# kvas7andy/unreal

Hardware: AMD Instinct MI355X
Metric: env-steps/sec (whole node), UNREAL maze 84x84 (higher is better)
Workload: dtype f32 (fp16x2-split MFMA operands, fp32 accumulate)

## Files before the change

unreal_amd/csrc/gemm_split.hip:

```cpp
#include "common.h"

namespace {

constexpr int BK = 32;
constexpr int NPL = 2;
typedef _Float16 f16x8 __attribute__((ext_vector_type(8)));
typedef _Float16 f16x2 __attribute__((ext_vector_type(2)));
constexpr int ROW_B = 80;
constexpr int FLAG_RELU = 1, FLAG_ACCUM = 2, FLAG_ATOMIC = 4, FLAG_RELU_MASK = 8, FLAG_RELU_BITS = 16;

typedef float f32x2 __attribute__((ext_vector_type(2)));
typedef unsigned int u32x2 __attribute__((ext_vector_type(2)));
typedef unsigned int u32x4 __attribute__((ext_vector_type(4)));

__device__ __forceinline__ int row_deal(int j) { return (j & ~7) | ((j & 1) << 2) | ((j >> 1) & 3); }

struct SplitArgs {
  int M, N, K;
  const float* A; int lda;
  const unsigned short* W; int ldw; long plane;
  float* C; int ldc;
  const float* bias;
  const float* mask; int ldm;
  int flags;
  int vecA;
  int nbx, nby;
  int splitk, ktiles_per_split;
  long slab_stride;
  const float* c_prev; float* c_out; float* h_out; int ld_h;
  const float* A2; int lda2, K1, K1pad;
  const float* dh_above; float* dc_io; const float* gates_act; const float* c_new; float* dpre;
  const float* a_absmax; float a_floor; const float* w_absmax; float* c_absmax0; float* c_absmax1;
};

template <int ROWS, bool VEC>
__device__ __forceinline__ f32x4 a_piece_load(const float* __restrict__ P, int ld, int rows_total, int K, int r0, int k0, int p,
                                              int tid) {
  const int id = tid + 256 * p;
  const int r = min(r0 + row_deal(id / (BK / 4)), rows_total - 1);
  const int k = k0 + (id % (BK / 4)) * 4;
  const float* row = P + (size_t)r * ld;
  if (VEC) return *reinterpret_cast<const f32x4*>(row + min(k, ld - 4));
  f32x4 v;
#pragma unroll
  for (int e = 0; e < 4; ++e) v[e] = row[min(k + e, K - 1)];
  return v;
}

__device__ __forceinline__ void split4_terms(float x0, float x1, float x2, float x3, u32x2 (&pl)[NPL]) {
  const f16x2 h01 = __builtin_convertvector((f32x2){x0, x1}, f16x2), h23 = __builtin_convertvector((f32x2){x2, x3}, f16x2);
  const f32x2 r01 = (f32x2){x0, x1} - __builtin_convertvector(h01, f32x2), r23 = (f32x2){x2, x3} - __builtin_convertvector(h23, f32x2);
  const f16x2 l01 = __builtin_convertvector(r01, f16x2), l23 = __builtin_convertvector(r23, f16x2);
  pl[0] = (u32x2){__builtin_bit_cast(unsigned int, h01), __builtin_bit_cast(unsigned int, h23)};
  pl[1] = (u32x2){__builtin_bit_cast(unsigned int, l01), __builtin_bit_cast(unsigned int, l23)};
}

template <int ROWS>
__device__ __forceinline__ void a_piece_store(unsigned char* S, f32x4 v, int klim, int p, int tid, float scale) {
  const int id = tid + 256 * p;
  const int r = row_deal(id / (BK / 4)), k = (id % (BK / 4)) * 4;
#pragma unroll
  for (int e = 0; e < 4; ++e) v[e] = k + e < klim ? v[e] * scale : 0.f;
  u32x2 pl[NPL];
  split4_terms(v[0], v[1], v[2], v[3], pl);
#pragma unroll
  for (int t = 0; t < NPL; ++t)
    *reinterpret_cast<u32x2*>(S + (t * ROWS + r) * ROW_B + k * 2) = pl[t];
}

template <int ROWS>
__device__ __forceinline__ u32x4 w_piece_load(const unsigned short* __restrict__ W, int ldw, long plane, int rows_total,
                                              int r0, int k0, int p, int tid) {
  const int id = tid + 256 * p;
  const int t = id / (ROWS * 4), r = row_deal((id / 4) % ROWS), c = id % 4;
  const int row = min(r0 + r, rows_total - 1);
  return *reinterpret_cast<const u32x4*>(W + t * plane + (size_t)row * ldw + k0 + c * 8);
}

template <int ROWS>
__device__ __forceinline__ void w_piece_store(unsigned char* S, u32x4 v, int p, int tid) {
  const int id = tid + 256 * p;
  const int t = id / (ROWS * 4), r = row_deal((id / 4) % ROWS), c = id % 4;
  *reinterpret_cast<u32x4*>(S + (t * ROWS + r) * ROW_B + c * 16) = v;
}

template <int BM, int BN, bool SWZ = false>
__device__ __forceinline__ void read_frags(const unsigned char* As, const unsigned char* Bs, int wm, int wn, int li, int kh,
                                           int ks, f16x8 (&af)[BM / 64][NPL], f16x8 (&bf)[BN / 64][NPL]) {
  const int c = 2 * ks + kh;
#pragma unroll
  for (int i = 0; i < BM / 64; ++i)
#pragma unroll
    for (int t = 0; t < NPL; ++t) {
      const int r = wm * (BM / 2) + i * 32 + li;
      af[i][t] = *reinterpret_cast<const f16x8*>(As + (t * BM + r) * ROW_B + (SWZ ? (c ^ ((r >> 4) & 3)) : c) * 16);
    }
#pragma unroll
  for (int j = 0; j < BN / 64; ++j)
#pragma unroll
    for (int t = 0; t < NPL; ++t) {
      const int r = wn * (BN / 2) + j * 32 + li;
      bf[j][t] = *reinterpret_cast<const f16x8*>(Bs + (t * BN + r) * ROW_B + (SWZ ? (c ^ ((r >> 4) & 3)) : c) * 16);
    }
}

template <int TM, int TN>
__device__ __forceinline__ void mma_frags(const f16x8 (&af)[TM][NPL], const f16x8 (&bf)[TN][NPL], f32x16 (&acc)[TM][TN]) {
#pragma unroll
  for (int i = 0; i < TM; ++i)
#pragma unroll
    for (int j = 0; j < TN; ++j) {
      f32x16 c = acc[i][j];
      c = __builtin_amdgcn_mfma_f32_32x32x16_f16(af[i][1], bf[j][0], c, 0, 0, 0);
      c = __builtin_amdgcn_mfma_f32_32x32x16_f16(af[i][0], bf[j][1], c, 0, 0, 0);
      c = __builtin_amdgcn_mfma_f32_32x32x16_f16(af[i][0], bf[j][0], c, 0, 0, 0);
      acc[i][j] = c;
    }
}

template <bool DUAL>
struct ASrc { const float* P; int ld, K, k0; };

template <bool DUAL>
__device__ __forceinline__ ASrc<DUAL> a_src(const SplitArgs& p, int kg) {
  ASrc<DUAL> s;
  if (DUAL) {
    const bool second = kg >= p.K1pad;
    s.P = second ? p.A2 : p.A; s.ld = second ? p.lda2 : p.lda;
    s.K = second ? p.K - p.K1pad : p.K1; s.k0 = second ? kg - p.K1pad : kg;
  } else {
    s.P = p.A; s.ld = p.lda; s.K = p.K; s.k0 = kg;
  }
  return s;
}

template <int BM, int BN, bool VEC, int EPI = 0, int KW = 1, bool DUAL = false>
__global__ __launch_bounds__(256 * KW, KW == 1 ? ((BM == 128 && EPI == 0) ? 3 : 2) : 1) void gemm_split_nt_kernel(SplitArgs p) {
  constexpr bool DEEP = BM == 64;
  constexpr int TM = BM / 64, TN = BN / 64;
  constexpr int PA = BM * BK / 1024, PW = NPL * BN / 64;
  constexpr int A_BYTES = NPL * BM * ROW_B, B_BYTES = NPL * BN * ROW_B;
  const float SA = pow2_scale(fmaxf(p.a_absmax ? *p.a_absmax : 0.f, p.a_floor));
  const float INV_A = pow2_inv(SA);
  const float INV_W = pow2_inv(pow2_scale(*p.w_absmax));
  constexpr bool HALF = BM == 128 && EPI == 0 && KW == 1;
  constexpr int C_BYTES = (HALF ? BM / 2 : BM) * (BN + 4) * 4;
  constexpr int OP_BYTES = A_BYTES + B_BYTES;
  constexpr int RED_BYTES = 64;
  constexpr int SMEM = OP_BYTES > (C_BYTES + RED_BYTES) ? OP_BYTES : (C_BYTES + RED_BYTES);
  static_assert(4 * KW * 4 <= RED_BYTES, "one float per wave");
  __shared__ __attribute__((aligned(16))) unsigned char smem_all[KW * SMEM];
  const int tid = KW == 1 ? (int)threadIdx.x : (int)(threadIdx.x & 255);
  const int grp = KW == 1 ? 0 : (int)(threadIdx.x >> 8);
  unsigned char* smem = smem_all + grp * SMEM;
  unsigned char* As = smem;
  unsigned char* Bs = smem + A_BYTES;

  const int L = blockIdx.x, xcd = L & 7, s = L >> 3;
  const int slab = s % p.splitk, s2 = s / p.splitk;
  const int bx = s2 % p.nbx, by = (s2 / p.nbx) * 8 + xcd;
  if (by >= p.nby) return;
  const int m0 = by * BM, n0 = bx * BN;
  if (EPI == 0) p.C += (size_t)slab * p.slab_stride;
  const int kt_base = slab * p.ktiles_per_split;
  const int nkt = min((p.K + BK - 1) / BK - kt_base, p.ktiles_per_split);
  if (nkt <= 0) return;
  const int lane = tid & 63, wave = tid >> 6;
  const int wm = wave >> 1, wn = wave & 1;
  const int li = lane & 31, kh = lane >> 5;

  f32x16 acc[TM][TN];
#pragma unroll
  for (int i = 0; i < TM; ++i)
#pragma unroll
    for (int j = 0; j < TN; ++j)
#pragma unroll
      for (int r = 0; r < 16; ++r) acc[i][j][r] = 0.f;

  f32x4 ra[2][PA];
  u32x4 rw[PW];
  const int shift = (int)((unsigned)by * 7u % (unsigned)nkt);
#define KT_AT(i) (kt_base + (((i) + shift) >= nkt ? (i) + shift - nkt : (i) + shift))
#define KG_AT(i) (KT_AT(min((i) * KW + grp, nkt - 1)) * BK)
#define KLIM(i, src) ((KW == 1 || (i) * KW + grp < nkt) ? (src).K - (src).k0 : 0)
#define A_LOAD(src, q) a_piece_load<BM, VEC>((src).P, (src).ld, p.M, (src).K, m0, (src).k0, q, tid)
  const int nit = (nkt + KW - 1) / KW;
  {
    const int k0 = KG_AT(0);
    const ASrc<DUAL> s0 = a_src<DUAL>(p, k0);
#pragma unroll
    for (int q = 0; q < PA; ++q) ra[0][q] = A_LOAD(s0, q);
#pragma unroll
    for (int q = 0; q < PW; ++q) rw[q] = w_piece_load<BN>(p.W, p.ldw, p.plane, p.N, n0, k0, q, tid);
#pragma unroll
    for (int q = 0; q < PA; ++q) a_piece_store<BM>(As, ra[0][q], KLIM(0, s0), q, tid, SA);
#pragma unroll
    for (int q = 0; q < PW; ++q) w_piece_store<BN>(Bs, rw[q], q, tid);
    const int k1 = KG_AT(1), k2 = KG_AT(2);
    const ASrc<DUAL> s1 = a_src<DUAL>(p, k1), s2_ = a_src<DUAL>(p, k2);
#pragma unroll
    for (int q = 0; q < PA; ++q) ra[0][q] = A_LOAD(s1, q);
    if (DEEP) {
#pragma unroll
      for (int q = 0; q < PA; ++q) ra[1][q] = A_LOAD(s2_, q);
    }
#pragma unroll
    for (int q = 0; q < PW; ++q) rw[q] = w_piece_load<BN>(p.W, p.ldw, p.plane, p.N, n0, k1, q, tid);
  }
  __syncthreads();

#define SPLIT_NT_TILE(S, IT)                                                                                        \
  {                                                                                                                 \
    f16x8 af[TM][NPL], bf[TN][NPL];                                                                                 \
    read_frags<BM, BN>(As, Bs, wm, wn, li, kh, 0, af, bf);                                                          \
    mma_frags<TM, TN>(af, bf, acc);                                                                                 \
    read_frags<BM, BN>(As, Bs, wm, wn, li, kh, 1, af, bf);          \
    __syncthreads();                                                               \
    const int kcur = KG_AT((IT) + 1), kw = KG_AT((IT) + 2), ka = KG_AT((IT) + (DEEP ? 3 : 2));                      \
    const ASrc<DUAL> scur = a_src<DUAL>(p, kcur), snext = a_src<DUAL>(p, ka);                                       \
    const int klim = KLIM((IT) + 1, scur);                                                                          \
    _Pragma("unroll") for (int q = 0; q < PA; ++q) {                                                                \
      a_piece_store<BM>(As, ra[S][q], klim, q, tid, SA);                                                            \
      ra[S][q] = A_LOAD(snext, q);                                                                                  \
    }                                                                                                               \
    _Pragma("unroll") for (int q = 0; q < PW; ++q) {                                                                \
      w_piece_store<BN>(Bs, rw[q], q, tid);                                                                         \
      rw[q] = w_piece_load<BN>(p.W, p.ldw, p.plane, p.N, n0, kw, q, tid);                                           \
    }                                                                                                               \
    mma_frags<TM, TN>(af, bf, acc);                                                                                 \
    __syncthreads();                                                                    \
  }
  if (DEEP) {
    for (int it = 0; it < nit; it += 2) {
      SPLIT_NT_TILE(0, it)
      if (it + 1 < nit) SPLIT_NT_TILE(1, it + 1)
    }
  } else {
    for (int it = 0; it < nit; ++it) SPLIT_NT_TILE(0, it)
  }
#undef SPLIT_NT_TILE
#undef A_LOAD
#undef KLIM
#undef KG_AT
#undef KT_AT

  if (EPI == 0 && (p.flags & FLAG_ATOMIC)) {
#pragma unroll
    for (int i = 0; i < TM; ++i)
#pragma unroll
      for (int j = 0; j < TN; ++j) {
        const int col = n0 + wn * (BN / 2) + j * 32 + li;
        if (col >= p.N) continue;
        const float bv = (p.bias && slab == 0 && grp == 0) ? p.bias[col] : 0.f;
#pragma unroll
        for (int r = 0; r < 16; ++r) {
          const int row = m0 + wm * (BM / 2) + i * 32 + (r & 3) + 8 * (r >> 2) + 4 * kh;
          const float v = (acc[i][j][r] * INV_A) * INV_W;
          if (row < p.M) atomicAdd(p.C + (size_t)row * p.ldc + col, v + bv);
        }
      }
    return;
  }
  constexpr int CLD = BN + 4;
  float* Cs = reinterpret_cast<float*>(smem);
  if (HALF) {
    const uint16_t* mbits = reinterpret_cast<const uint16_t*>(p.mask);
    const bool vecC = ((p.ldc & 3) == 0) && ((((uintptr_t)p.C) & 15) == 0) &&
                      (!p.bias || ((((uintptr_t)p.bias) & 15) == 0)) &&
                      (!(p.flags & FLAG_RELU_MASK) || (((p.ldm & 3) == 0) && ((((uintptr_t)p.mask) & 15) == 0)));
    constexpr int CV = BN / 4;
    float omax = 0.f;
#pragma unroll 1
    for (int half = 0; half < 2; ++half) {
      if (half) __syncthreads();
      if (wm == half) {
#pragma unroll
        for (int i = 0; i < TM; ++i)
#pragma unroll
          for (int j = 0; j < TN; ++j)
#pragma unroll
            for (int r = 0; r < 16; ++r)
              Cs[(i * 32 + (r & 3) + 8 * (r >> 2) + 4 * kh) * CLD + wn * (BN / 2) + j * 32 + li] =
                  (acc[i][j][r] * INV_A) * INV_W;
      }
      __syncthreads();
      for (int id = threadIdx.x; id < (BM / 2) * CV; id += 256) {
        const int r = id / CV, c4 = (id % CV) * 4;
        const int row = m0 + half * (BM / 2) + r, col = n0 + c4;
        if (row >= p.M || col >= p.N) continue;
        f32x4 v = *reinterpret_cast<const f32x4*>(Cs + r * CLD + c4);
        float* cp = p.C + (size_t)row * p.ldc + col;
        if (vecC && col + 3 < p.N) {
          if (p.bias) { const f32x4 b4 = *reinterpret_cast<const f32x4*>(p.bias + col); v += b4; }
          if (p.flags & FLAG_ACCUM) v += *reinterpret_cast<const f32x4*>(cp);
          if (p.flags & FLAG_RELU) {
#pragma unroll
            for (int e = 0; e < 4; ++e) v[e] = fmaxf(v[e], 0.f);
          }
          if (p.flags & FLAG_RELU_MASK) {
            const f32x4 m4 = *reinterpret_cast<const f32x4*>(p.mask + (size_t)row * p.ldm + col);
#pragma unroll
            for (int e = 0; e < 4; ++e) v[e] = m4[e] > 0.f ? v[e] : 0.f;
          }
          if (p.flags & FLAG_RELU_BITS) {
            const unsigned w = mbits[(size_t)row * p.ldm + (col >> 4)] >> (col & 15);
#pragma unroll
            for (int e = 0; e < 4; ++e) v[e] = ((w >> e) & 1u) ? v[e] : 0.f;
          }
          *reinterpret_cast<f32x4*>(cp) = v;
          omax = fmaxf(fmaxf(omax, fmaxf(fabsf(v[0]), fabsf(v[1]))), fmaxf(fabsf(v[2]), fabsf(v[3])));
        } else {
#pragma unroll
          for (int e = 0; e < 4; ++e) {
            if (col + e >= p.N) break;
            float x = v[e] + (p.bias ? p.bias[col + e] : 0.f);
            if (p.flags & FLAG_ACCUM) x += cp[e];
            if (p.flags & FLAG_RELU) x = fmaxf(x, 0.f);
            if (p.flags & FLAG_RELU_MASK) x = (p.mask[(size_t)row * p.ldm + col + e] > 0.f) ? x : 0.f;
            if (p.flags & FLAG_RELU_BITS) x = ((mbits[(size_t)row * p.ldm + ((col + e) >> 4)] >> ((col + e) & 15)) & 1u) ? x : 0.f;
            cp[e] = x;
            omax = fmaxf(omax, fabsf(x));
          }
        }
      }
    }
    if (p.c_absmax0) {
      __syncthreads();
      float* wmx0 = reinterpret_cast<float*>(smem_all);
      omax = wave_max(omax);
      if ((threadIdx.x & 63) == 0) wmx0[threadIdx.x >> 6] = omax;
      __syncthreads();
      if (threadIdx.x < 64) absmax_commit(p.c_absmax0, fmaxf(fmaxf(wmx0[0], wmx0[1]), fmaxf(wmx0[2], wmx0[3])));
    }
    return;
  }
#pragma unroll
  for (int i = 0; i < TM; ++i)
#pragma unroll
    for (int j = 0; j < TN; ++j)
#pragma unroll
      for (int r = 0; r < 16; ++r)
        Cs[(wm * (BM / 2) + i * 32 + (r & 3) + 8 * (r >> 2) + 4 * kh) * CLD + wn * (BN / 2) + j * 32 + li] =
            (acc[i][j][r] * INV_A) * INV_W;
  __syncthreads();
  const float* C0 = reinterpret_cast<const float*>(smem_all);
  constexpr int GSTRIDE = SMEM / 4;
  if (EPI == 1) {
    const int u0 = bx * (BN / 4);
    const bool add_pre = (p.flags & FLAG_ACCUM) != 0;
    constexpr int ITEMS = BM * (BN / 4) / (256 * KW);
    float cprev[ITEMS], pre4[ITEMS][4];
#pragma unroll
    for (int e = 0; e < ITEMS; ++e) {
      const int id = threadIdx.x + e * 256 * KW;
      const int row = min(m0 + id / (BN / 4), p.M - 1), u = u0 + id % (BN / 4);
      cprev[e] = p.c_prev[(size_t)row * 256 + u];
#pragma unroll
      for (int g4 = 0; g4 < 4; ++g4) pre4[e][g4] = add_pre ? p.C[(size_t)row * p.ldc + g4 * 256 + u] : 0.f;
    }
    static_assert((256 * KW) % (BN / 4) == 0, "a lane keeps its hidden unit over the pairs it handles");
    float bb[4];
#pragma unroll
    for (int g4 = 0; g4 < 4; ++g4) bb[g4] = p.bias[g4 * 256 + u0 + threadIdx.x % (BN / 4)];
#pragma unroll
    for (int e = 0; e < ITEMS; ++e) {
      const int id = threadIdx.x + e * 256 * KW;
      const int r = id / (BN / 4), ul = id % (BN / 4);
      const int row = m0 + r, u = u0 + ul;
      const float* cs = C0 + r * CLD + (ul >> 4) * 64 + (ul & 15);
      float s4[4];
#pragma unroll
      for (int g4 = 0; g4 < 4; ++g4) {
        float a = cs[g4 * 16];
#pragma unroll
        for (int g = 1; g < KW; ++g) a += cs[g * GSTRIDE + g4 * 16];
        s4[g4] = add_pre ? a + pre4[e][g4] : a;
      }
      const float gi = 1.f / (1.f + expf(-(s4[0] + bb[0])));
      const float gj = tanhf(s4[1] + bb[1]);
      const float gf = 1.f / (1.f + expf(-(s4[2] + bb[2] + 1.0f)));
      const float go = 1.f / (1.f + expf(-(s4[3] + bb[3])));
      const float c = cprev[e] * gf + gi * gj;
      if (row >= p.M) continue;
      float* pre = p.C + (size_t)row * p.ldc;
      pre[u] = gi; pre[256 + u] = gj; pre[512 + u] = gf; pre[768 + u] = go;
      p.c_out[(size_t)row * 256 + u] = c;
      p.h_out[(size_t)row * p.ld_h + u] = tanhf(c) * go;
    }
    return;
  }
  if (EPI == 2) {
    constexpr int ITEMS = BM * BN / (256 * KW), CH = ITEMS < 4 ? ITEMS : 4;
    float omax = 0.f;
#pragma unroll
    for (int e0 = 0; e0 < ITEMS; e0 += CH) {
      float dha[CH], dcv[CH], cn[CH], cp[CH], ga[CH][4];
#pragma unroll
      for (int e = 0; e < CH; ++e) {
        const int id = threadIdx.x + (e0 + e) * 256 * KW;
        const size_t g = (size_t)min(m0 + id / BN, p.M - 1) * 256 + n0 + id % BN;
        dha[e] = p.dh_above[g]; dcv[e] = p.dc_io[g]; cn[e] = p.c_new[g]; cp[e] = p.c_prev[g];
#pragma unroll
        for (int g4 = 0; g4 < 4; ++g4) ga[e][g4] = p.gates_act[(g / 256) * 1024 + g4 * 256 + g % 256];
      }
#pragma unroll
      for (int e = 0; e < CH; ++e) {
        const int id = threadIdx.x + (e0 + e) * 256 * KW;
        const int r = id / BN, cidx = id % BN;
        float rec = C0[r * CLD + cidx];
#pragma unroll
        for (int g = 1; g < KW; ++g) rec += C0[g * GSTRIDE + r * CLD + cidx];
        if (m0 + r >= p.M) continue;
        const size_t g = (size_t)(m0 + r) * 256 + n0 + cidx;
        const float i = ga[e][0], j = ga[e][1], f = ga[e][2], o = ga[e][3];
        const float dh = dha[e] + rec;
        const float tc = tanhf(cn[e]);
        const float dc = dcv[e] + dh * o * (1.f - tc * tc);
        float* d = p.dpre + (g / 256) * 1024 + g % 256;
        const float d0 = dc * j * i * (1.f - i), d1 = dc * i * (1.f - j * j), d2 = dc * cp[e] * f * (1.f - f),
                    d3 = dh * tc * o * (1.f - o);
        d[0] = d0; d[256] = d1; d[512] = d2; d[768] = d3;
        omax = fmaxf(fmaxf(omax, fmaxf(fabsf(d0), fabsf(d1))), fmaxf(fabsf(d2), fabsf(d3)));
        p.dc_io[g] = dc * f;
      }
    }
    {
      float* wmx = reinterpret_cast<float*>(smem_all + C_BYTES);
      omax = wave_max(omax);
      if ((threadIdx.x & 63) == 0) wmx[threadIdx.x >> 6] = omax;
      __syncthreads();
      if (threadIdx.x < 64) {
        float m = wmx[0];
#pragma unroll
        for (int g = 1; g < 4 * KW; ++g) m = fmaxf(m, wmx[g]);
        absmax_commit(p.c_absmax0, m);
        absmax_commit(p.c_absmax1, m);
      }
    }
    return;
  }
  const uint16_t* mbits = reinterpret_cast<const uint16_t*>(p.mask);
  const bool vecC = ((p.ldc & 3) == 0) && ((((uintptr_t)p.C) & 15) == 0) &&
                    (!p.bias || ((((uintptr_t)p.bias) & 15) == 0)) &&
                    (!(p.flags & FLAG_RELU_MASK) || (((p.ldm & 3) == 0) && ((((uintptr_t)p.mask) & 15) == 0)));
  constexpr int CV = BN / 4;
  float omax = 0.f;
  static_assert((BM * CV) % (256 * KW) == 0, "every lane makes the same number of passes (absmax_commit needs whole waves)");
  for (int id = threadIdx.x; id < BM * CV; id += 256 * KW) {
    const int r = id / CV, c4 = (id % CV) * 4;
    const int row = m0 + r, col = n0 + c4;
    if (row >= p.M || col >= p.N) continue;
    f32x4 v = *reinterpret_cast<const f32x4*>(C0 + r * CLD + c4);
#pragma unroll
    for (int g = 1; g < KW; ++g) v += *reinterpret_cast<const f32x4*>(C0 + g * GSTRIDE + r * CLD + c4);
    float* cp = p.C + (size_t)row * p.ldc + col;
    if (vecC && col + 3 < p.N) {
      if (p.bias) { const f32x4 b4 = *reinterpret_cast<const f32x4*>(p.bias + col); v += b4; }
      if (p.flags & FLAG_ACCUM) v += *reinterpret_cast<const f32x4*>(cp);
      if (p.flags & FLAG_RELU) {
#pragma unroll
        for (int e = 0; e < 4; ++e) v[e] = fmaxf(v[e], 0.f);
      }
      if (p.flags & FLAG_RELU_MASK) {
        const f32x4 m4 = *reinterpret_cast<const f32x4*>(p.mask + (size_t)row * p.ldm + col);
#pragma unroll
        for (int e = 0; e < 4; ++e) v[e] = m4[e] > 0.f ? v[e] : 0.f;
      }
      if (p.flags & FLAG_RELU_BITS) {
        const unsigned w = mbits[(size_t)row * p.ldm + (col >> 4)] >> (col & 15);
#pragma unroll
        for (int e = 0; e < 4; ++e) v[e] = ((w >> e) & 1u) ? v[e] : 0.f;
      }
      *reinterpret_cast<f32x4*>(cp) = v;
      omax = fmaxf(fmaxf(omax, fmaxf(fabsf(v[0]), fabsf(v[1]))), fmaxf(fabsf(v[2]), fabsf(v[3])));
    } else {
#pragma unroll
      for (int e = 0; e < 4; ++e) {
        if (col + e >= p.N) break;
        float x = v[e] + (p.bias ? p.bias[col + e] : 0.f);
        if (p.flags & FLAG_ACCUM) x += cp[e];
        if (p.flags & FLAG_RELU) x = fmaxf(x, 0.f);
        if (p.flags & FLAG_RELU_MASK) x = (p.mask[(size_t)row * p.ldm + col + e] > 0.f) ? x : 0.f;
        if (p.flags & FLAG_RELU_BITS) x = ((mbits[(size_t)row * p.ldm + ((col + e) >> 4)] >> ((col + e) & 15)) & 1u) ? x : 0.f;
        cp[e] = x;
        omax = fmaxf(omax, fabsf(x));
      }
    }
  }
  if (p.c_absmax0) {
    float* wmx0 = reinterpret_cast<float*>(smem_all + C_BYTES);
    omax = wave_max(omax);
    if ((threadIdx.x & 63) == 0) wmx0[threadIdx.x >> 6] = omax;
    __syncthreads();
    if (threadIdx.x < 64) {
      float m = wmx0[0];
#pragma unroll
      for (int g = 1; g < 4 * KW; ++g) m = fmaxf(m, wmx0[g]);
      absmax_commit(p.c_absmax0, m);
    }
  }
}

struct SplitTnArgs {
  int M, N, K;
  const float* A; int lda;
  const float* B; int ldb;
  float* C; int ldc;
  float* colsum;
  int ntx, nty, splitk, ktiles_per_split;
  const float* a_absmax; const float* b_absmax;
};

__device__ __forceinline__ int tn_m4() {
  const int t = threadIdx.x;
  return ((t >> 1) & 1) | (((t >> 4) & 1) << 1) | (((t >> 2) & 3) << 2) | (((t >> 5) & 1) << 4);
}
__device__ __forceinline__ int tn_k4() {
  const int t = threadIdx.x;
  return (t & 1) | ((t >> 6) << 1);
}

__device__ __forceinline__ void tn_piece_load(const float* __restrict__ P, int ld, int K, int c0, int k0, f32x4 (&reg)[4]) {
  const int m4 = tn_m4(), k4 = tn_k4();
  const int col = min(c0 + 4 * m4, ld - 4);
#pragma unroll
  for (int kk = 0; kk < 4; ++kk) {
    const int k = min(k0 + 4 * k4 + kk, K - 1);
    reg[kk] = *reinterpret_cast<const f32x4*>(P + (size_t)k * ld + col);
  }
}

template <int ROWS, bool RAGGED>
__device__ __forceinline__ void tn_piece_store(unsigned char* S, const f32x4 (&reg)[4], int klim, float scale) {
  const int m4 = tn_m4(), k4 = tn_k4();
  bool ok[4];
#pragma unroll
  for (int kk = 0; kk < 4; ++kk) ok[kk] = !RAGGED || 4 * k4 + kk < klim;
#pragma unroll
  for (int j = 0; j < 4; ++j) {
    const int r = 4 * m4 + j;
    u32x2 pl[NPL];
    split4_terms(ok[0] ? reg[0][j] * scale : 0.f, ok[1] ? reg[1][j] * scale : 0.f, ok[2] ? reg[2][j] * scale : 0.f,
                 ok[3] ? reg[3][j] * scale : 0.f, pl);
    const int off = (((k4 >> 1) ^ ((r >> 4) & 3)) * 2 + (k4 & 1)) * 8;
#pragma unroll
    for (int t = 0; t < NPL; ++t)
      *reinterpret_cast<u32x2*>(S + (t * ROWS + r) * ROW_B + off) = pl[t];
  }
}

template <bool RAGGED>
__device__ __forceinline__ void tn_colsum_acc(const f32x4 (&reg)[4], int klim, float w, float (&cs)[4]) {
  const int k4 = tn_k4();
#pragma unroll
  for (int kk = 0; kk < 4; ++kk) {
    const float wk = (!RAGGED || 4 * k4 + kk < klim) ? w : 0.f;
#pragma unroll
    for (int j = 0; j < 4; ++j) cs[j] = fmaf(wk, reg[kk][j], cs[j]);
  }
}

template <bool RAGGED>
__global__ __launch_bounds__(256, 2) void gemm_split_tn_kernel(SplitTnArgs p) {
  constexpr int BM = 128, BN = 128, TM = 2, TN = 2;
  constexpr int A_BYTES = NPL * BM * ROW_B, B_BYTES = NPL * BN * ROW_B;
  constexpr int OP_BYTES = A_BYTES + B_BYTES;
  __shared__ __attribute__((aligned(16))) unsigned char smem[OP_BYTES > 8 * BN * 4 ? OP_BYTES : 8 * BN * 4];
  const float SA = pow2_scale(*p.a_absmax), SB = pow2_scale(*p.b_absmax);
  const float INV_A = pow2_inv(SA), INV_B = pow2_inv(SB);
  unsigned char* As = smem;
  unsigned char* Bs = smem + A_BYTES;

  const int L = blockIdx.x, xcd = L & 7, s = L >> 3;
  const int tiles = p.ntx * p.nty;
  const int slab = (s / tiles) * 8 + xcd, tile = s % tiles;
  if (slab >= p.splitk) return;
  const int bx = tile % p.ntx, by = tile / p.ntx;
  const int m0 = by * BM, n0 = bx * BN;
  const int nk_total = (p.K + BK - 1) / BK;
  const int kt0 = slab * p.ktiles_per_split, kt1 = min(nk_total, kt0 + p.ktiles_per_split);
  if (kt0 >= kt1) return;
  const int nkt = kt1 - kt0;
  const int lane = threadIdx.x & 63, wave = threadIdx.x >> 6;
  const int wm = wave >> 1, wn = wave & 1;
  const int li = lane & 31, kh = lane >> 5;

  f32x16 acc[TM][TN];
#pragma unroll
  for (int i = 0; i < TM; ++i)
#pragma unroll
    for (int j = 0; j < TN; ++j)
#pragma unroll
      for (int r = 0; r < 16; ++r) acc[i][j][r] = 0.f;

  constexpr int TN_FLUSH = 8;
  f32x16 tot[TM][TN];
#pragma unroll
  for (int i = 0; i < TM; ++i)
#pragma unroll
    for (int j = 0; j < TN; ++j)
#pragma unroll
      for (int r = 0; r < 16; ++r) tot[i][j][r] = 0.f;
  f32x4 ra[4], rb[4];
  const float csw = (p.colsum != nullptr && by == 0) ? 1.f : 0.f;
  float cs[4] = {0.f, 0.f, 0.f, 0.f};
  tn_piece_load(p.A, p.lda, p.K, m0, kt0 * BK, ra);
  tn_piece_load(p.B, p.ldb, p.K, n0, kt0 * BK, rb);
  tn_piece_store<BM, RAGGED>(As, ra, p.K - kt0 * BK, SA);
  tn_piece_store<BN, RAGGED>(Bs, rb, p.K - kt0 * BK, SB);
  tn_colsum_acc<RAGGED>(rb, p.K - kt0 * BK, csw, cs);
  {
    const int k1 = (kt0 + min(1, nkt - 1)) * BK;
    tn_piece_load(p.A, p.lda, p.K, m0, k1, ra);
    tn_piece_load(p.B, p.ldb, p.K, n0, k1, rb);
  }
  __syncthreads();

  for (int it = 0; it < nkt; ++it) {
    f16x8 af[TM][NPL], bf[TN][NPL];
    read_frags<BM, BN, true>(As, Bs, wm, wn, li, kh, 0, af, bf);
    mma_frags<TM, TN>(af, bf, acc);
    read_frags<BM, BN, true>(As, Bs, wm, wn, li, kh, 1, af, bf);
    __syncthreads();
    const int kcur = (kt0 + min(it + 1, nkt - 1)) * BK, knext = (kt0 + min(it + 2, nkt - 1)) * BK;
    tn_piece_store<BM, RAGGED>(As, ra, p.K - kcur, SA);
    tn_piece_load(p.A, p.lda, p.K, m0, knext, ra);
    tn_piece_store<BN, RAGGED>(Bs, rb, p.K - kcur, SB);
    tn_colsum_acc<RAGGED>(rb, p.K - kcur, (it + 1 < nkt) ? csw : 0.f, cs);
    tn_piece_load(p.B, p.ldb, p.K, n0, knext, rb);
    mma_frags<TM, TN>(af, bf, acc);
    if ((it + 1) % TN_FLUSH == 0) {
#pragma unroll
      for (int i = 0; i < TM; ++i)
#pragma unroll
        for (int j = 0; j < TN; ++j)
#pragma unroll
          for (int r = 0; r < 16; ++r) { tot[i][j][r] += acc[i][j][r]; acc[i][j][r] = 0.f; }
    }
    __syncthreads();
  }
#pragma unroll
  for (int i = 0; i < TM; ++i)
#pragma unroll
    for (int j = 0; j < TN; ++j)
#pragma unroll
      for (int r = 0; r < 16; ++r) acc[i][j][r] += tot[i][j][r];

  if (csw != 0.f) {
    float* red = reinterpret_cast<float*>(smem);
    const int m4 = tn_m4(), k4 = tn_k4();
#pragma unroll
    for (int j = 0; j < 4; ++j) red[k4 * BN + 4 * m4 + j] = cs[j];
    __syncthreads();
    if (threadIdx.x < BN && n0 + threadIdx.x < p.N) {
      float v = 0.f;
#pragma unroll
      for (int k = 0; k < 8; ++k) v += red[k * BN + threadIdx.x];
      atomicAdd(p.colsum + n0 + threadIdx.x, v);
    }
  }
#pragma unroll
  for (int i = 0; i < TM; ++i)
#pragma unroll
    for (int j = 0; j < TN; ++j) {
      const int col = n0 + wn * (BN / 2) + j * 32 + li;
      if (col >= p.N) continue;
#pragma unroll
      for (int r = 0; r < 16; ++r) {
        const int row = m0 + wm * (BM / 2) + i * 32 + (r & 3) + 8 * (r >> 2) + 4 * kh;
        if (row < p.M) atomicAdd(p.C + (size_t)row * p.ldc + col, (acc[i][j][r] * INV_A) * INV_B);
      }
    }
}

__global__ __launch_bounds__(256) void split_planes_f16x2_kernel(int rows, int cols, const float* __restrict__ src, int ld_src,
                                                                 int transpose, unsigned short* __restrict__ dst, int ld_dst,
                                                                 long plane, int row_perm, const float* __restrict__ w_absmax) {
  __shared__ float t[32][33];
  const float sw = pow2_scale(*w_absmax);
  const int c0 = blockIdx.x * 32, r0 = blockIdx.y * 32;
  const int tx = threadIdx.x & 31, ty = threadIdx.x >> 5;
  for (int y = ty; y < 32; y += 8)
    if (r0 + y < rows && c0 + tx < cols) t[y][tx] = src[(size_t)(r0 + y) * ld_src + c0 + tx];
  __syncthreads();
  for (int y = ty; y < 32; y += 8) {
    int orow = transpose ? c0 + y : r0 + y;
    const int ocol = transpose ? r0 + tx : c0 + tx;
    if (row_perm == 1) orow = ((orow & 255) >> 4) * 64 + (orow >> 8) * 16 + (orow & 15);
    const bool ok = transpose ? (c0 + y < cols && r0 + tx < rows) : (r0 + y < rows && c0 + tx < cols);
    if (!ok) continue;
    const float x = (transpose ? t[tx][y] : t[y][tx]) * sw;
    const _Float16 h = (_Float16)x;
    const _Float16 l = (_Float16)(x - (float)h);
    dst[(size_t)orow * ld_dst + ocol] = __builtin_bit_cast(unsigned short, h);
    dst[plane + (size_t)orow * ld_dst + ocol] = __builtin_bit_cast(unsigned short, l);
  }
}

__global__ __launch_bounds__(256) void absmax_kernel(int rows, int cols, const float* __restrict__ x, int ld, float* slot) {
  float m = 0.f;
  if (ld == cols && (cols & 3) == 0 && ((((uintptr_t)x) & 15) == 0)) {
    const long n4 = (long)rows * cols / 4;
    const f32x4* x4 = reinterpret_cast<const f32x4*>(x);
    for (long i = (long)blockIdx.x * 256 + threadIdx.x; i < n4; i += (long)gridDim.x * 256) {
      const f32x4 v = x4[i];
      m = fmaxf(fmaxf(m, fmaxf(fabsf(v[0]), fabsf(v[1]))), fmaxf(fabsf(v[2]), fabsf(v[3])));
    }
  } else {
    const int wave = (blockIdx.x * 256 + threadIdx.x) >> 6, nw = (gridDim.x * 256) >> 6, lane = threadIdx.x & 63;
    for (int r = wave; r < rows; r += nw)
      for (int c = lane; c < cols; c += 64) m = fmaxf(m, fabsf(x[(size_t)r * ld + c]));
  }
  __shared__ float wm[4];
  m = wave_max(m);
  if ((threadIdx.x & 63) == 0) wm[threadIdx.x >> 6] = m;
  __syncthreads();
  if (threadIdx.x < 64) absmax_commit(slot, fmaxf(fmaxf(wm[0], wm[1]), fmaxf(wm[2], wm[3])));
}

struct MultiAbsDesc { const float* src; float* wmax; long n; long block0; };
struct MultiSplitDesc { const float* src; unsigned short* dst; const float* wmax; long rows, cols, ld_src, transpose, row_perm, ld_dst, plane, tiles_x, block0; };

__global__ __launch_bounds__(256) void multi_absmax_kernel(const MultiAbsDesc* __restrict__ descs, int n_desc) {
  int d = 0;
  while (d + 1 < n_desc && (long)blockIdx.x >= descs[d + 1].block0) ++d;
  const MultiAbsDesc D = descs[d];
  const long e0 = ((long)blockIdx.x - D.block0) * 8192, e1 = min(D.n, e0 + 8192);
  float m = 0.f;
  for (long i = e0 + threadIdx.x; i < e1; i += 256) m = fmaxf(m, fabsf(D.src[i]));
  __shared__ float wm[4];
  m = wave_max(m);
  if ((threadIdx.x & 63) == 0) wm[threadIdx.x >> 6] = m;
  __syncthreads();
  if (threadIdx.x < 64) absmax_commit(D.wmax, fmaxf(fmaxf(wm[0], wm[1]), fmaxf(wm[2], wm[3])));
}

__global__ __launch_bounds__(256) void multi_split_kernel(const MultiSplitDesc* __restrict__ descs, int n_desc) {
  int d = 0;
  while (d + 1 < n_desc && (long)blockIdx.x >= descs[d + 1].block0) ++d;
  const MultiSplitDesc D = descs[d];
  __shared__ float t[32][33];
  const float sw = pow2_scale(*D.wmax);
  const long tile = (long)blockIdx.x - D.block0;
  const int c0 = (int)(tile % D.tiles_x) * 32, r0 = (int)(tile / D.tiles_x) * 32;
  const int rows = (int)D.rows, cols = (int)D.cols;
  const int tx = threadIdx.x & 31, ty = threadIdx.x >> 5;
  for (int y = ty; y < 32; y += 8)
    if (r0 + y < rows && c0 + tx < cols) t[y][tx] = D.src[(size_t)(r0 + y) * D.ld_src + c0 + tx];
  __syncthreads();
  for (int y = ty; y < 32; y += 8) {
    int orow = D.transpose ? c0 + y : r0 + y;
// ... 310 lines not shown
```

Measured before the change: 3.780 million.

## Add specialized batched epilogue for full interior GEMM tiles

Adds a fast epilogue path for full, aligned tiles that is templated on the mask mode and the accumulate flag. It hoists the bias load and precomputes 32-bit byte offsets, then issues batched prefetches of the C, mask and bit-mask rows ahead of the LDS reads. In the half-tile mode it can also fetch the bitmask for both halves up front. The aim is to remove per-element branching and bounds checks and to overlap global loads with the shared-memory reduction, at the cost of more registers, code size and six template instantiations per kernel.

```diff
diff --git a/unreal_amd/csrc/gemm_split.hip b/unreal_amd/csrc/gemm_split.hip
--- a/unreal_amd/csrc/gemm_split.hip
+++ b/unreal_amd/csrc/gemm_split.hip
@@ -132,6 +132,120 @@
     s.P = p.A; s.ld = p.lda; s.K = p.K; s.k0 = kg;
   }
   return s;
+}
+
+constexpr int epi_nb(int trips, int mk, bool acc) { return (mk == 1 && acc && trips > 4) ? 4 : trips; }
+
+template <int CV, int NB, int MK, bool ACC>
+__device__ __forceinline__ void epi_fetch(const SplitArgs& p, int rowu, int col0, unsigned oc, unsigned om, f32x4 (&rc)[NB],
+                                          f32x4 (&rm)[NB], unsigned (&rw)[NB]) {
+  constexpr int RSTEP = 256 / CV;
+#pragma unroll
+  for (int e = 0; e < NB; ++e) {
+    const size_t row = (size_t)(rowu + e * RSTEP);
+    if (ACC) rc[e] = *reinterpret_cast<const f32x4*>(reinterpret_cast<const char*>(p.C + row * p.ldc + col0) + oc);
+    if (MK == 1) rm[e] = *reinterpret_cast<const f32x4*>(reinterpret_cast<const char*>(p.mask + row * p.ldm + col0) + om);
+    if (MK == 2)
+      rw[e] = *reinterpret_cast<const uint16_t*>(
+          reinterpret_cast<const char*>(reinterpret_cast<const uint16_t*>(p.mask) + row * p.ldm + (col0 >> 4)) + om);
+  }
+}
+
+template <int CV, int CLD, int NB, int MK, bool ACC>
+__device__ __forceinline__ void epi_apply(const float* cs, int sh, f32x4 b4, bool relu, const f32x4 (&rc)[NB],
+                                          const f32x4 (&rm)[NB], const unsigned (&rw)[NB], f32x4 (&v)[NB], float& omax) {
+  constexpr int RSTEP = 256 / CV;
+#pragma unroll
+  for (int e = 0; e < NB; ++e) {
+    v[e] = *reinterpret_cast<const f32x4*>(cs + e * RSTEP * CLD) + b4;
+    if (ACC) v[e] += rc[e];
+#pragma unroll
+    for (int k = 0; k < 4; ++k) {
+      v[e][k] = relu ? fmaxf(v[e][k], 0.f) : v[e][k];
+      if (MK == 1) v[e][k] = rm[e][k] > 0.f ? v[e][k] : 0.f;
+      if (MK == 2) v[e][k] = ((rw[e] >> (sh + k)) & 1u) ? v[e][k] : 0.f;
+    }
+    omax = fmaxf(fmaxf(omax, fmaxf(fabsf(v[e][0]), fabsf(v[e][1]))), fmaxf(fabsf(v[e][2]), fabsf(v[e][3])));
+  }
+}
+
+template <int CV, int NB>
+__device__ __forceinline__ void epi_store(const SplitArgs& p, int rowu, int col0, unsigned oc, const f32x4 (&v)[NB]) {
+  constexpr int RSTEP = 256 / CV;
+#pragma unroll
+  for (int e = 0; e < NB; ++e)
+    *reinterpret_cast<f32x4*>(reinterpret_cast<char*>(p.C + (size_t)(rowu + e * RSTEP) * p.ldc + col0) + oc) = v[e];
+}
+
+template <int BM, int BN, int NH, int MK, bool ACC>
+__device__ __forceinline__ float epi_fast(const SplitArgs& p, float* Cs, const f32x16 (&acc)[BM / 64][BN / 64], int m0, int n0) {
+  constexpr int CV = BN / 4, CLD = BN + 4, RSTEP = 256 / CV, TRIPS = (BM / NH) * CV / 256, NB = epi_nb(TRIPS, MK, ACC);
+  static_assert(256 % CV == 0 && TRIPS % NB == 0, "a lane keeps its columns; whole batches");
+  const int lane = threadIdx.x & 63, wave = threadIdx.x >> 6;
+  const int wm = wave >> 1, wn = wave & 1, li = lane & 31, kh = lane >> 5;
+  const int fr = threadIdx.x / CV, c4 = (threadIdx.x % CV) * 4;
+  const unsigned oc = ((unsigned)fr * p.ldc + c4) * 4u;
+  const unsigned om = MK == 1 ? ((unsigned)fr * p.ldm + c4) * 4u : ((unsigned)fr * p.ldm + (c4 >> 4)) * 2u;
+  const bool relu = (p.flags & FLAG_RELU) != 0;
+  f32x4 b4 = {-0.f, -0.f, -0.f, -0.f};
+  if (p.bias) b4 = *reinterpret_cast<const f32x4*>(p.bias + n0 + c4);
+  f32x4 rc[NB], rm[NB];
+  unsigned rw[NB], rw1[NB];
+  float omax = 0.f;
+  constexpr bool AHEAD = MK == 2 && !ACC && NH == 2;
+#pragma unroll 1
+  for (int h = 0; h < NH; ++h) {
+    if (h) __syncthreads();
+    const int rowu = m0 + h * (BM / NH);
+    if (!AHEAD) epi_fetch<CV, NB, MK, ACC>(p, rowu, n0, oc, om, rc, rm, rw);
+    if (AHEAD && h == 0) {
+      epi_fetch<CV, NB, MK, ACC>(p, m0, n0, oc, om, rc, rm, rw);
+      epi_fetch<CV, NB, MK, ACC>(p, m0 + BM / NH, n0, oc, om, rc, rm, rw1);
+    }
+    if (AHEAD && h) {
+#pragma unroll
+      for (int e = 0; e < NB; ++e) rw[e] = rw1[e];
+    }
+    if (NH == 1 || wm == h) {
+#pragma unroll
+      for (int i = 0; i < BM / 64; ++i)
+#pragma unroll
+        for (int j = 0; j < BN / 64; ++j)
+#pragma unroll
+          for (int r = 0; r < 16; ++r)
+            Cs[((NH == 1 ? wm * (BM / 2) : 0) + i * 32 + (r & 3) + 8 * (r >> 2) + 4 * kh) * CLD + wn * (BN / 2) + j * 32 + li] =
+                acc[i][j][r];
+    }
+    __syncthreads();
+#pragma unroll
+    for (int t = 0; t < TRIPS; t += NB) {
+      f32x4 v[NB];
+      if (t) epi_fetch<CV, NB, MK, ACC>(p, rowu + t * RSTEP, n0, oc, om, rc, rm, rw);
+      epi_apply<CV, CLD, NB, MK, ACC>(Cs + (fr + t * RSTEP) * CLD + c4, c4 & 15, b4, relu, rc, rm, rw, v, omax);
+      epi_store<CV, NB>(p, rowu + t * RSTEP, n0, oc, v);
+    }
+  }
+  return omax;
+}
+
+template <int BM, int BN, int NH>
+__device__ __forceinline__ float epi_fast_dispatch(const SplitArgs& p, float* Cs, f32x16 (&acc)[BM / 64][BN / 64],
+                                                   float inv_a, float inv_w, int m0, int n0) {
+#pragma unroll
+  for (int i = 0; i < BM / 64; ++i)
+#pragma unroll
+    for (int j = 0; j < BN / 64; ++j)
+#pragma unroll
+      for (int r = 0; r < 16; ++r) acc[i][j][r] = (acc[i][j][r] * inv_a) * inv_w;
+  const int mk = (p.flags & FLAG_RELU_MASK) ? 1 : (p.flags & FLAG_RELU_BITS) ? 2 : 0;
+  switch (mk + ((p.flags & FLAG_ACCUM) ? 3 : 0)) {
+    case 0: return epi_fast<BM, BN, NH, 0, false>(p, Cs, acc, m0, n0);
+    case 1: return epi_fast<BM, BN, NH, 1, false>(p, Cs, acc, m0, n0);
+    case 2: return epi_fast<BM, BN, NH, 2, false>(p, Cs, acc, m0, n0);
+    case 3: return epi_fast<BM, BN, NH, 0, true>(p, Cs, acc, m0, n0);
+    case 4: return epi_fast<BM, BN, NH, 1, true>(p, Cs, acc, m0, n0);
+    default: return epi_fast<BM, BN, NH, 2, true>(p, Cs, acc, m0, n0);
+  }
 }
 
 template <int BM, int BN, bool VEC, int EPI = 0, int KW = 1, bool DUAL = false>
@@ -270,8 +384,10 @@
                       (!(p.flags & FLAG_RELU_MASK) || (((p.ldm & 3) == 0) && ((((uintptr_t)p.mask) & 15) == 0)));
     constexpr int CV = BN / 4;
     float omax = 0.f;
+    const bool fast = vecC && m0 + BM <= p.M && n0 + BN <= p.N && (p.ldc | p.ldm) < (1 << 26);
+    if (fast) omax = epi_fast_dispatch<BM, BN, 2>(p, Cs, acc, INV_A, INV_W, m0, n0);
 #pragma unroll 1
-    for (int half = 0; half < 2; ++half) {
+    for (int half = fast ? 2 : 0; half < 2; ++half) {
       if (half) __syncthreads();
       if (wm == half) {
 #pragma unroll
@@ -334,15 +450,24 @@
     }
     return;
   }
-#pragma unroll
-  for (int i = 0; i < TM; ++i)
-#pragma unroll
-    for (int j = 0; j < TN; ++j)
-#pragma unroll
-      for (int r = 0; r < 16; ++r)
-        Cs[(wm * (BM / 2) + i * 32 + (r & 3) + 8 * (r >> 2) + 4 * kh) * CLD + wn * (BN / 2) + j * 32 + li] =
-            (acc[i][j][r] * INV_A) * INV_W;
-  __syncthreads();
+  const bool vecC = ((p.ldc & 3) == 0) && ((((uintptr_t)p.C) & 15) == 0) &&
+                    (!p.bias || ((((uintptr_t)p.bias) & 15) == 0)) &&
+                    (!(p.flags & FLAG_RELU_MASK) || (((p.ldm & 3) == 0) && ((((uintptr_t)p.mask) & 15) == 0)));
+  const bool fast = EPI == 0 && KW == 1 && vecC && m0 + BM <= p.M && n0 + BN <= p.N && (p.ldc | p.ldm) < (1 << 26);
+  float omax = 0.f;
+  if (fast) {
+    omax = epi_fast_dispatch<BM, BN, 1>(p, Cs, acc, INV_A, INV_W, m0, n0);
+  } else {
+#pragma unroll
+    for (int i = 0; i < TM; ++i)
+#pragma unroll
+      for (int j = 0; j < TN; ++j)
+#pragma unroll
+        for (int r = 0; r < 16; ++r)
+          Cs[(wm * (BM / 2) + i * 32 + (r & 3) + 8 * (r >> 2) + 4 * kh) * CLD + wn * (BN / 2) + j * 32 + li] =
+              (acc[i][j][r] * INV_A) * INV_W;
+    __syncthreads();
+  }
   const float* C0 = reinterpret_cast<const float*>(smem_all);
   constexpr int GSTRIDE = SMEM / 4;
   if (EPI == 1) {
@@ -440,13 +565,9 @@
     return;
   }
   const uint16_t* mbits = reinterpret_cast<const uint16_t*>(p.mask);
-  const bool vecC = ((p.ldc & 3) == 0) && ((((uintptr_t)p.C) & 15) == 0) &&
-                    (!p.bias || ((((uintptr_t)p.bias) & 15) == 0)) &&
-                    (!(p.flags & FLAG_RELU_MASK) || (((p.ldm & 3) == 0) && ((((uintptr_t)p.mask) & 15) == 0)));
   constexpr int CV = BN / 4;
-  float omax = 0.f;
   static_assert((BM * CV) % (256 * KW) == 0, "every lane makes the same number of passes (absmax_commit needs whole waves)");
-  for (int id = threadIdx.x; id < BM * CV; id += 256 * KW) {
+  for (int id = fast ? BM * CV : threadIdx.x; id < BM * CV; id += 256 * KW) {
     const int r = id / CV, c4 = (id % CV) * 4;
     const int row = m0 + r, col = n0 + c4;
     if (row >= p.M || col >= p.N) continue;
```

Measured after the change: 3.808 million, median of 6. About the same (+0.7%).
